# whwh747/A-Low-Texture-Robust-Hybrid-Feature-Based-Visual-Odometry

Measured on AMD Instinct MI355X. Metric: RGB-D frames/sec (640×480, 1k ORB + LSD + PEAC) at 1/2/4/8 GPUs, higher is better.
Workload: dtype u8/u16 integer + f32/f64; 1 GPU; 640x480 synthetic RGB-D, 1000 ORB (quota; 3/4 std + 1/4 lowtex scenes) + LSD lines + PEAC planes, 8192 frames per GPU per step (std640); frames_per_gpu=8192, parallelism=frames sharded, 1 rank(s), no data-path collective, distinct_frames=256, resident_bytes_per_frame_estimate=21100000

## Files before the change

### a-low-texture-robust-hybrid-feature-based-visual-odometry_amd/csrc/orb_level.hip

```cpp
#include "hvo_internal.hpp"
#include <string.h>
#include <algorithm>
#include <vector>

#define LT_TP 64
#define LT_ND (LT_TP / 4)
#define LT_TR 46
#define LT_MAXO 40
#define LT_CAND 368
#define LT_PEND 328
#define LT_TABN 48

typedef unsigned short lt_us2 __attribute__((ext_vector_type(2)));

struct __attribute__((aligned(16))) LtWave {
    uint32_t T[LT_TR * LT_ND];
    union {
        struct { uint8_t S[LT_TR * LT_TP]; unsigned short cand[LT_CAND]; unsigned short pend[LT_PEND]; unsigned long long mk_min[8], mk_ini[8]; } f;
        uint32_t V[((LT_TR + 1) / 2) * LT_MAXO];
    } u;
    int tab[4][LT_TABN];
};
static_assert(sizeof(LtWave) <= 8192, "five workgroups per CU");

struct LevelArgs {
    const uint8_t *rd; size_t rd_stride;
    uint8_t *wr; size_t wr_stride;
    uint8_t *blur; size_t blur_stride;
    LevelGeom L, D; int has_next;
    const OrbTile *tiles; int ntiles, tpw, groups, nframes;
    const int *xofs, *xalpha, *yofs, *ybeta;
    uint32_t *cell_kp; int *cell_cnt; int ncells, iniTh, minTh; int *flags;
    int k0, k1, k2, k3;
    int res_dw;
    int skip;
};

static __device__ __forceinline__ int lt_reflect(int p, int n)
{
    if (p < 0) p = -p;
    if (p >= n) p = 2 * (n - 1) - p;
    return p < 0 ? 0 : p;
}
static __device__ __forceinline__ int lt_mbcnt(unsigned long long m)
{
    return __builtin_amdgcn_mbcnt_hi((unsigned)(m >> 32), __builtin_amdgcn_mbcnt_lo((unsigned)m, 0u));
}

static __device__ __forceinline__ int lt_min3(int a, int b, int c) { int r; asm("v_min3_i32 %0, %1, %2, %3" : "=v"(r) : "v"(a), "v"(b), "v"(c)); return r; }
static __device__ __forceinline__ int lt_max3(int a, int b, int c) { int r; asm("v_max3_i32 %0, %1, %2, %3" : "=v"(r) : "v"(a), "v"(b), "v"(c)); return r; }

static __device__ __forceinline__ int lt_fast_score(const uint8_t *p, int v)
{
    constexpr int tp = LT_TP;
    int r[16];
    r[0] = p[3 * tp];    r[1] = p[3 * tp + 1];   r[2] = p[2 * tp + 2];   r[3] = p[tp + 3];
    r[4] = p[3];         r[5] = p[-tp + 3];      r[6] = p[-2 * tp + 2];  r[7] = p[-3 * tp + 1];
    r[8] = p[-3 * tp];   r[9] = p[-3 * tp - 1];  r[10] = p[-2 * tp - 2]; r[11] = p[-tp - 3];
    r[12] = p[-3];       r[13] = p[tp - 3];      r[14] = p[2 * tp - 2];  r[15] = p[3 * tp - 1];
    int d[16], e[16], a3[16], b3[16];
#pragma unroll
    for (int k = 0; k < 16; k++) { d[k] = v - r[k]; e[k] = r[k] - v; }
#pragma unroll
    for (int k = 0; k < 16; k++) { a3[k] = lt_min3(d[k], d[(k + 1) & 15], d[(k + 2) & 15]); b3[k] = lt_min3(e[k], e[(k + 1) & 15], e[(k + 2) & 15]); }
    int best = -1000;
#pragma unroll
    for (int k = 0; k < 16; k++)
        best = lt_max3(best, lt_min3(a3[k], a3[(k + 3) & 15], a3[(k + 6) & 15]), lt_min3(b3[k], b3[(k + 3) & 15], b3[(k + 6) & 15]));
    return best - 1;
}

static __device__ __forceinline__ void lt_row_sums(unsigned W0, unsigned W1, unsigned W2, unsigned klo, unsigned khi, unsigned hs[4])
{
    const unsigned A0 = __builtin_amdgcn_alignbyte(W1, W0, 1), B0 = __builtin_amdgcn_alignbyte(W2, W1, 1);
    const unsigned A1 = __builtin_amdgcn_alignbyte(W1, W0, 2), B1 = __builtin_amdgcn_alignbyte(W2, W1, 2);
    const unsigned A2 = __builtin_amdgcn_alignbyte(W1, W0, 3), B2 = __builtin_amdgcn_alignbyte(W2, W1, 3);
    hs[0] = __builtin_amdgcn_udot4(A0, klo, __builtin_amdgcn_udot4(B0, khi, 0u, false), false);
    hs[1] = __builtin_amdgcn_udot4(A1, klo, __builtin_amdgcn_udot4(B1, khi, 0u, false), false);
    hs[2] = __builtin_amdgcn_udot4(A2, klo, __builtin_amdgcn_udot4(B2, khi, 0u, false), false);
    hs[3] = __builtin_amdgcn_udot4(W1, klo, __builtin_amdgcn_udot4(W2, khi, 0u, false), false);
}
static __device__ __forceinline__ unsigned lt_dot2(unsigned a, unsigned w, unsigned c)
{
    return __builtin_amdgcn_udot2(__builtin_bit_cast(lt_us2, a), __builtin_bit_cast(lt_us2, w), c, false);
}

template <int NW>
__global__ __launch_bounds__(64 * NW, 5) void k_orb_level(const LevelArgs A)
{
    __shared__ LtWave lds_[NW];
    const int wv = threadIdx.x >> 6, lane = threadIdx.x & 63;
    const int xcd = blockIdx.x & 7, q = blockIdx.x >> 3;
    const int fr8 = q / A.groups, g = q - fr8 * A.groups;
    const int frame = fr8 * 8 + xcd;
    if (frame >= A.nframes) return;
    LtWave &W = lds_[wv];
    const LevelGeom &L = A.L;
    const uint8_t *img = A.rd + (size_t)frame * A.rd_stride;
    uint8_t *bdst = A.blur + (size_t)frame * A.blur_stride;
    const uint8_t *T8 = reinterpret_cast<const uint8_t *>(W.T);
    const unsigned long long ltm = (1ull << lane) - 1ull;

    for (int ti = 0; ti < A.tpw; ti++) {
        const int tidx = (g * A.tpw + ti) * NW + wv;
        if (tidx >= A.ntiles) break;
        const OrbTile t = A.tiles[tidx];
        const int lx0 = t.bx0 - 4, ly0 = t.by0 - 3;
        const int rows = t.bh + 6;
        const int xr = max(t.fx0 + t.fw, t.bx0 + t.bw) + 3;
        __builtin_amdgcn_wave_barrier();
        {
            typedef uint32_t lt_u4 __attribute__((ext_vector_type(4), aligned(4)));
            uint4 v[3];
#pragma unroll
            for (int k = 0; k < 3; k++) {
                const int i = lane + 64 * k, r = i >> 2, c = i & 3;
                v[k] = make_uint4(0, 0, 0, 0);
                if (r < rows) {
                    const int y = lt_reflect(ly0 + r, L.h);
                    const lt_u4 q4 = *reinterpret_cast<const lt_u4 *>(img + (size_t)y * L.pitch + lx0 + 16 * c);
                    v[k] = make_uint4(q4.x, q4.y, q4.z, q4.w);
                }
            }
            int tb0 = 0, tb1 = 0, tb2 = 0, tb3 = 0;
            const bool want_tab = A.has_next && lane < LT_TABN;
            if (want_tab) {
                const int dx = min(t.dxa + lane, A.D.w - 1), dy = min(t.dya + lane, A.D.h - 1);
                tb0 = A.xofs[dx]; tb1 = A.xalpha[dx]; tb2 = A.yofs[dy]; tb3 = A.ybeta[dy];
            }
#pragma unroll
            for (int k = 0; k < 3; k++) {
                const int i = lane + 64 * k;
                if ((i >> 2) < rows) reinterpret_cast<uint4 *>(W.T)[i] = v[k];
            }
            if (want_tab) { W.tab[0][lane] = tb0; W.tab[1][lane] = tb1; W.tab[2][lane] = tb2; W.tab[3][lane] = tb3; }
        }
        if (lx0 < 0) {
            if (lane < rows) { const unsigned d1 = W.T[lane * LT_ND + 1]; W.T[lane * LT_ND] = __builtin_amdgcn_perm(d1, d1, 0x01020300u); }
        }
        if (xr > L.w) {
            uint8_t *Tb = reinterpret_cast<uint8_t *>(W.T);
            if (lane < rows) {
                const int c = L.w - lx0;
#pragma unroll
                for (int k = 0; k < 3; k++) if (L.w + k < xr) Tb[lane * LT_TP + c + k] = Tb[lane * LT_TP + c - 2 - k];
            }
        }
        __builtin_amdgcn_wave_barrier();

        if (t.fw > 0 && !(A.skip & 1)) {
            uint8_t *S = W.u.f.S;
            {
                uint4 *Sz = reinterpret_cast<uint4 *>(S);
                const int nz = (rows * LT_TP + 15) >> 4;
                for (int i = lane; i < nz; i += 64) Sz[i] = make_uint4(0, 0, 0, 0);
            }
            const int cx0 = t.fx0 - lx0, cx1 = cx0 + t.fw, ih = t.bh, iw = t.fw, P = iw * ih;
            const int dws = cx0 >> 2, nd = ((cx1 - 1) >> 2) - dws + 1, items = ih * nd;
            const int rcp = (65536 + nd - 1) / nd;
            const int minTh = A.minTh;
            int ncand = 0, npend = 0;
            auto rest = [&](const unsigned short *pp, int cnt) {
                int pass = 0, xy = 0;
                if (lane < cnt) {
                    xy = pp[lane];
                    const uint8_t *qq = T8 + (xy >> 8) * LT_TP + (xy & 0xFF);
                    const int v = qq[0];
#define LT_PMN(o) min((int)qq[o], (int)qq[-(o)])
#define LT_PMX(o) max((int)qq[o], (int)qq[-(o)])
                    const int n0 = LT_PMN(3 * LT_TP), n1 = LT_PMN(3), n2 = LT_PMN(2 * LT_TP + 2), n3 = LT_PMN(-2 * LT_TP + 2);
                    const int n4 = LT_PMN(3 * LT_TP + 1), n5 = LT_PMN(LT_TP + 3), n6 = LT_PMN(-LT_TP + 3), n7 = LT_PMN(-3 * LT_TP + 1);
                    const int x0 = LT_PMX(3 * LT_TP), x1 = LT_PMX(3), x2 = LT_PMX(2 * LT_TP + 2), x3 = LT_PMX(-2 * LT_TP + 2);
                    const int x4 = LT_PMX(3 * LT_TP + 1), x5 = LT_PMX(LT_TP + 3), x6 = LT_PMX(-LT_TP + 3), x7 = LT_PMX(-3 * LT_TP + 1);
#undef LT_PMN
#undef LT_PMX
                    const int M1 = lt_max3(lt_max3(n0, n1, n2), lt_max3(n3, n4, n5), max(n6, n7));
                    const int M2 = lt_min3(lt_min3(x0, x1, x2), lt_min3(x3, x4, x5), min(x6, x7));
                    pass = (int)(M1 < v - minTh) | (int)(M2 > v + minTh);
                }
                const unsigned long long m = __ballot(pass != 0);
                const int p = ncand + __popcll(m & ltm);
                if (pass && p < LT_CAND) W.u.f.cand[p] = (unsigned short)xy;
                ncand += __popcll(m);
            };
            for (int base = 0; base < items; base += 64) {
                const int it = base + lane;
                const int ok = it < items;
                const int itc = ok ? it : 0;
                const int r = (itc * rcp) >> 16, dwi = dws + itc - r * nd;
                const unsigned t4 = W.T[r * LT_ND + dwi], v4 = W.T[(r + 3) * LT_ND + dwi], b4 = W.T[(r + 6) * LT_ND + dwi];
                const int xb = 4 * dwi;
                const int jl = max(cx0 - xb, 0), jh = min(cx1 - xb, 4);
                const unsigned inm = ok ? (((1u << jh) - 1u) & ~((1u << jl) - 1u)) : 0u;
                int pj[4];
#pragma unroll
                for (int j = 0; j < 4; j++) {
                    const int v = (v4 >> (8 * j)) & 0xFF, tt = (t4 >> (8 * j)) & 0xFF, bb = (b4 >> (8 * j)) & 0xFF;
                    pj[j] = (int)((inm >> j) & 1u) & ((int)(min(tt, bb) < v - minTh) | (int)(max(tt, bb) > v + minTh));
                }
                const unsigned long long m0 = __ballot(pj[0] != 0), m1 = __ballot(pj[1] != 0), m2 = __ballot(pj[2] != 0), m3 = __ballot(pj[3] != 0);
                if ((m0 | m1 | m2 | m3) != 0ull) {
                    const int p0 = npend + lt_mbcnt(m0) + lt_mbcnt(m1) + lt_mbcnt(m2) + lt_mbcnt(m3);
                    const int p1 = p0 + pj[0], p2 = p1 + pj[1], p3 = p2 + pj[2];
                    const int yx = ((r + 3) << 8) | xb;
                    W.u.f.pend[pj[0] ? p0 : LT_PEND - 1] = (unsigned short)yx;
                    W.u.f.pend[pj[1] ? p1 : LT_PEND - 1] = (unsigned short)(yx + 1);
                    W.u.f.pend[pj[2] ? p2 : LT_PEND - 1] = (unsigned short)(yx + 2);
                    W.u.f.pend[pj[3] ? p3 : LT_PEND - 1] = (unsigned short)(yx + 3);
                    npend += __popcll(m0) + __popcll(m1) + __popcll(m2) + __popcll(m3);
                    int head = 0;
                    while (npend - head >= 64) { rest(W.u.f.pend + head, 64); head += 64; }
                    if (head) {
                        const int left = npend - head;
                        const int tv = W.u.f.pend[head + (lane < left ? lane : 0)];
                        if (lane < left) W.u.f.pend[lane] = (unsigned short)tv;
                        npend = left;
                    }
                }
            }
            if (npend > 0) rest(W.u.f.pend, npend);
            __builtin_amdgcn_wave_barrier();
            const uint8_t *T0 = T8 + 3 * LT_TP + cx0;
            uint8_t *S0 = S + 3 * LT_TP + cx0;
            if (ncand <= LT_CAND) {
                for (int i = lane; i < ncand; i += 64) {
                    const int xy = W.u.f.cand[i], o = (xy >> 8) * LT_TP + (xy & 0xFF);
                    const int s = lt_fast_score(T8 + o, T8[o]);
                    S[o] = (uint8_t)(s >= minTh ? s : 0);
                }
            } else {
                for (int p = lane; p < P; p += 64) {
                    const int y = p / iw, x = p - y * iw;
                    const int s = lt_fast_score(T0 + y * LT_TP + x, T0[y * LT_TP + x]);
                    S0[y * LT_TP + x] = (uint8_t)(s >= minTh ? s : 0);
                }
            }
            __builtin_amdgcn_wave_barrier();
            uint32_t *out = A.cell_kp + ((size_t)frame * A.ncells + t.cell) * HVO_CELL_CAP;
            const int ex = lx0 - L.minBX, ey = ly0 - L.minBY;
            int n_ini = 0, pos = 0;
            if (ncand <= LT_CAND) {
                int st = 0;
                for (int base = 0; base < ncand; base += 64, st++) {
                    const int i = base + lane;
// ... 121 lines not shown
                for (int i = 0; i < 4; i++) {
                    sxo[i] = W.tab[0][4 * c + i] - lx0;
                    a01[i] = (unsigned)W.tab[1][4 * c + i];
                }
                const int wbase = sxo[0] >> 2;
                unsigned sel = 0;
#pragma unroll
                for (int i = 0; i < 4; i++) sel |= (unsigned)((sxo[i] - 4 * wbase) & 7) << (8 * i);
                auto hrow = [&](int sy, unsigned tt[4]) {
                    if (A.res_dw) {
                        const uint32_t *rp = W.T + (sy - ly0) * LT_ND + wbase;
                        const uint32_t w0 = rp[0], w1 = rp[1], w2 = rp[2];
                        const uint32_t Lb = __builtin_amdgcn_perm(w1, w0, sel);
                        const uint32_t Rb = __builtin_amdgcn_perm(__builtin_amdgcn_alignbyte(w2, w1, 1), __builtin_amdgcn_alignbyte(w1, w0, 1), sel);
                        tt[0] = lt_dot2(__builtin_amdgcn_perm(Rb, Lb, 0x0c040c00u), a01[0], 0u);
                        tt[1] = lt_dot2(__builtin_amdgcn_perm(Rb, Lb, 0x0c050c01u), a01[1], 0u);
                        tt[2] = lt_dot2(__builtin_amdgcn_perm(Rb, Lb, 0x0c060c02u), a01[2], 0u);
                        tt[3] = lt_dot2(__builtin_amdgcn_perm(Rb, Lb, 0x0c070c03u), a01[3], 0u);
                    } else {
                        const uint8_t *rp = T8 + (sy - ly0) * LT_TP;
#pragma unroll
                        for (int i = 0; i < 4; i++) {
                            const int sx = min(max(sxo[i], 0), LT_TP - 2);
                            tt[i] = lt_dot2((unsigned)rp[sx] | ((unsigned)rp[sx + 1] << 16), a01[i], 0u);
                        }
                    }
                };
#pragma unroll
                for (int rr = 0; rr < RG; rr++) {
                    const int dyu = t.dya + gr * RG + rr, dy = min(dyu, t.dyb - 1);
                    const int yo = W.tab[2][dy - t.dya], sy0 = yo & 0xFFFF, sy1 = yo >> 16;
                    const unsigned yb = (unsigned)W.tab[3][dy - t.dya];
                    const unsigned b0 = yb & 0xFFFFu, b1 = yb >> 16;
                    unsigned t0[4], t1[4];
                    hrow(sy0, t0);
                    hrow(sy1, t1);
                    uint32_t ov = 0;
#pragma unroll
                    for (int i = 0; i < 4; i++) {
                        const unsigned v = ((__umul24(b0, t0[i] >> 4) >> 16) + (__umul24(b1, t1[i] >> 4) >> 16) + 2u) >> 2;
                        ov |= (v & 0xFFu) << (8 * i);
                    }
                    if (dyu < t.dyb) *reinterpret_cast<uint32_t *>(dst + (size_t)dy * D.pitch + dxq) = ov;
                }
            }
        }
    }
}

struct LtIv { int a, b, idx; };

static void lt_split(std::vector<LtIv> &v, int a, int b, int align)
{
    if (b <= a) return;
    const int len = b - a, n = (len + LT_MAXO - 1) / LT_MAXO;
    int step = (len + n - 1) / n;
    step = (step + align - 1) / align * align;
    for (int s = a; s < b; s += step) v.push_back({ s, std::min(s + step, b), -1 });
}

bool orb_level_build(OrbPlan &P, const std::vector<CellDesc> &cells, const std::vector<int> &xofs, const std::vector<int> &yofs, std::vector<OrbTile> &tiles)
{
    tiles.clear();
    for (int l = 0; l < P.nlevels; l++) {
        LevelGeom &L = P.lev[l];
        P.lt_off[l] = (int)tiles.size();
        std::vector<LtIv> cols, rws;
        for (int c = L.cell_off; c < L.cell_off + L.ncells; c++) {
            const CellDesc &cd = cells[c];
            const int fx = cd.x0 + 3, fxe = cd.x0 + cd.vw - 3, fy = cd.y0 + 3, fye = cd.y0 + cd.vh - 3;
            bool hc = false, hr = false;
            for (auto &iv : cols) hc |= iv.a == fx;
            for (auto &iv : rws) hr |= iv.a == fy;
            if (!hc) cols.push_back({ fx, fxe, (int)cols.size() });
            if (!hr) rws.push_back({ fy, fye, (int)rws.size() });
        }
        if ((int)(cols.size() * rws.size()) != L.ncells) return false;
        for (size_t j = 1; j < cols.size(); j++) if (cols[j].a != cols[j - 1].b) return false;
        for (size_t i = 1; i < rws.size(); i++) if (rws[i].a != rws[i - 1].b) return false;
        const int W4 = (L.w + 3) & ~3;
        std::vector<LtIv> xs, ys;
        if (cols.empty()) { lt_split(xs, 0, W4, 4); lt_split(ys, 0, L.h, 1); }
        else {
            lt_split(xs, 0, cols[0].a & ~3, 4);
            for (size_t j = 0; j < cols.size(); j++) {
                const int a = cols[j].a & ~3, b = (j + 1 < cols.size() ? cols[j + 1].a : cols[j].b) & ~3;
                xs.push_back({ a, b, (int)j });
            }
            lt_split(xs, cols.back().b & ~3, W4, 4);
            lt_split(ys, 0, rws[0].a, 1);
            for (size_t i = 0; i < rws.size(); i++) ys.push_back({ rws[i].a, rws[i].b, (int)i });
            lt_split(ys, rws.back().b, L.h, 1);
        }
        const bool has_next = l + 1 < P.nlevels;
        const int *xo = has_next ? xofs.data() + P.lev[l + 1].rs_off : nullptr;
        const int *yo = has_next ? yofs.data() + P.lev[l + 1].ry_off : nullptr;
        const int dw = has_next ? P.lev[l + 1].w : 0, dh = has_next ? P.lev[l + 1].h : 0;
        for (auto &iy : ys) for (auto &ix : xs) {
            OrbTile t; memset(&t, 0, sizeof(t));
            t.bx0 = (short)ix.a; t.bw = (short)(ix.b - ix.a); t.by0 = (short)iy.a; t.bh = (short)(iy.b - iy.a);
            t.cell = -1; t.fx0 = (short)ix.a; t.fw = 0;
            if (ix.idx >= 0 && iy.idx >= 0) {
                t.fx0 = (short)cols[ix.idx].a; t.fw = (short)(cols[ix.idx].b - cols[ix.idx].a);
                t.cell = (short)(L.cell_off + iy.idx * (int)cols.size() + ix.idx);
                const CellDesc &cd = cells[t.cell];
                if (cd.x0 + 3 != t.fx0 || cd.y0 + 3 != t.by0 || cd.vh - 6 != t.bh || cd.vw - 6 != t.fw) return false;
            }
            if (t.bh < 1 || (t.bw < 1 && t.fw < 1)) continue;
            const int xr = std::max(t.fx0 + t.fw, t.bx0 + t.bw) + 3;
            if (t.bw > LT_MAXO || t.bh > LT_MAXO || t.bh + 6 > LT_TR || xr - (t.bx0 - 4) > LT_TP || (t.bw & 3) || (t.bx0 & 3)) return false;
            if (t.fw > 0 && ((t.fw * t.bh + 3) / 4 > LT_CAND + 1000)) return false;
            int dxa = 0, dxb = 0, dya = 0, dyb = 0;
            if (has_next && t.bw > 0) {
                const int dw4 = (dw + 3) & ~3;
                while (dxa < dw4 && xo[std::min(dxa, dw - 1)] < t.bx0) dxa += 4;
                dxb = dxa; while (dxb < dw4 && xo[std::min(dxb, dw - 1)] < t.bx0 + t.bw) dxb += 4;
                while (dya < dh && (yo[dya] & 0xFFFF) < t.by0) dya++;
                dyb = dya; while (dyb < dh && (yo[dyb] & 0xFFFF) < t.by0 + t.bh) dyb++;
                for (int dx = dxa; dx < std::min(dxb, dw); dx++) if (xo[dx] + 1 - (t.bx0 - 4) > LT_TP - 1) return false;
            }
            if (dxb - dxa > LT_TABN || dyb - dya > LT_TABN) return false;
            t.dxa = (short)dxa; t.dxb = (short)dxb; t.dya = (short)dya; t.dyb = (short)dyb;
            tiles.push_back(t);
        }
        P.lt_cnt[l] = (int)tiles.size() - P.lt_off[l];
    }
    return true;
}

int orb_level_run(hvo_ctx *ctx, int c0, int n, hipStream_t st, int k0, int k1, int k2, int k3)
{
    OrbPlan &P = ctx->orb;
    for (int l = 0; l < P.nlevels; l++) {
        LevelArgs A;
        A.L = P.lev[l]; A.has_next = l + 1 < P.nlevels; A.D = P.lev[A.has_next ? l + 1 : l];
        if (l == 0) { A.rd = P.d_pyr + (size_t)c0 * P.pyr_bytes; A.rd_stride = P.pyr_bytes; } else { A.rd = P.d_lvl + A.L.lvl_off; A.rd_stride = P.lvl_bytes; }
        A.wr = P.d_lvl + A.D.lvl_off; A.wr_stride = P.lvl_bytes;
        A.blur = P.d_blur + A.L.img_off; A.blur_stride = P.blur_bytes;
        A.tiles = P.d_ltiles + P.lt_off[l]; A.ntiles = P.lt_cnt[l];
        const int nw = P.lt_nw;
        A.tpw = P.lt_tpw; A.groups = (A.ntiles + nw * A.tpw - 1) / (nw * A.tpw); A.nframes = n;
        A.xofs = P.d_rs_xofs + A.D.rs_off; A.xalpha = P.d_rs_xalpha + A.D.rs_off; A.yofs = P.d_rs_yofs + A.D.ry_off; A.ybeta = P.d_rs_ybeta + A.D.ry_off;
        A.cell_kp = P.d_cell_kp; A.cell_cnt = P.d_cell_cnt; A.ncells = P.ncells; A.iniTh = ctx->p.orb_ini_th_fast; A.minTh = ctx->p.orb_min_th_fast;
        A.res_dw = A.has_next && P.resize_dw[l + 1];
#ifdef HVO_TIMING_KNOBS
        A.skip = getenv("HVO_LT_SKIP") ? atoi(getenv("HVO_LT_SKIP")) : 0;
#else
        A.skip = 0;
#endif
        if (ctx->readings & HVO_READING_BLUR_FLOAT) A.skip |= 2;
        A.flags = P.d_flags + c0; A.k0 = k0; A.k1 = k1; A.k2 = k2; A.k3 = k3;
        if (A.ntiles < 1) continue;
        const int n8 = (n + 7) / 8 * 8;
        if (nw == 1) hipLaunchKernelGGL(k_orb_level<1>, dim3((unsigned)(n8 * A.groups)), dim3(64), 0, st, A);
        else if (nw == 2) hipLaunchKernelGGL(k_orb_level<2>, dim3((unsigned)(n8 * A.groups)), dim3(128), 0, st, A);
        else hipLaunchKernelGGL(k_orb_level<4>, dim3((unsigned)(n8 * A.groups)), dim3(256), 0, st, A);
    }
    return HVO_OK;
}
```

### a-low-texture-robust-hybrid-feature-based-visual-odometry_amd/csrc/peac_slots.inc

```

struct SlDec { int p, K, D, code, moff, mB, r0, r1; };
struct __attribute__((aligned(16))) SlLds { double ps[4][16]; LendRed red[4]; LendWin win[4]; SlDec dec[4]; int ncnt[4]; };
#define SL_SLOT(x) ((x) & 0xFFFF)
#define SL_PACK(label, slot) (((label) << 16) | (slot))

static __device__ __forceinline__ void row_min16x2(double (&k)[2], int (&i)[2])
{
    double g[2] = { k[0], k[1] };
#pragma unroll
    for (int s_ = 0; s_ < 4; s_++) {
        double t[2];
#pragma unroll
        for (int n = 0; n < 2; n++) t[n] = dpp_f64(g[n], g[n], s_);
#pragma unroll
        for (int n = 0; n < 2; n++) g[n] = key_min(t[n], g[n]);
    }
    int c[2];
#pragma unroll
    for (int n = 0; n < 2; n++) c[n] = (k[n] == g[n]) ? i[n] : 0x7FFFFFFF;
#pragma unroll
    for (int s_ = 0; s_ < 4; s_++) {
#pragma unroll
        for (int n = 0; n < 2; n++) { const int t = dpp_i32(c[n], c[n], s_); c[n] = min(c[n], t); }
    }
#pragma unroll
    for (int n = 0; n < 2; n++) { k[n] = g[n]; i[n] = c[n]; }
}

struct TQUpdateS {
    double kk[2], mk[2], kn[2]; int li[2], mi[2], x[2], ln[2], nx;
    __device__ __forceinline__ void issue(const TQueue &Q, const int *lq, int rl, int nx_, int x0, double k0, int l0, int x1, double k1, int l1)
    {
        nx = nx_; x[0] = x0; x[1] = x1; kn[0] = k0; kn[1] = k1; ln[0] = l0; ln[1] = l1;
#pragma unroll
        for (int t = 0; t < 2; t++) {
            kk[t] = TQ_INF; mk[t] = TQ_INF; mi[t] = 0x7FFFFFFF; li[t] = 0x7FFFFFFF;
            if (t < nx) { const int s = (x[t] & ~15) + rl; kk[t] = Q.K[s]; li[t] = lq[s]; const int j = ((x[t] >> 8) << 4) + rl; mk[t] = Q.M1k[j]; mi[t] = Q.M1i[j]; }
        }
    }
    __device__ __forceinline__ int take(const TQueue &Q, int *lq, int rl, bool writer)
    {
#pragma unroll
        for (int t = 0; t < 2; t++) if (writer && t < nx) { Q.K[x[t]] = kn[t]; lq[x[t]] = ln[t]; }
        double bk[2]; int bi[2];
#pragma unroll
        for (int t = 0; t < 2; t++) {
            double k = kk[t]; int i = li[t];
#pragma unroll
            for (int u = 0; u < 2; u++) if (u < nx && ((x[u] ^ x[t]) >> 4) == 0 && (x[u] & 15) == rl) { k = kn[u]; i = ln[u]; }
            if (t >= nx) { k = TQ_INF; i = 0x7FFFFFFF; }
            bk[t] = k; bi[t] = i;
        }
        row_min16x2(bk, bi);
#pragma unroll
        for (int t = 0; t < 2; t++) if (writer && t < nx) { Q.M1k[x[t] >> 4] = bk[t]; Q.M1i[x[t] >> 4] = bi[t]; }
        double sk[2]; int si[2];
#pragma unroll
        for (int t = 0; t < 2; t++) {
            double k = mk[t]; int i = mi[t];
#pragma unroll
            for (int u = 0; u < 2; u++) if (u < nx && ((x[u] ^ x[t]) >> 8) == 0 && ((x[u] >> 4) & 15) == rl) { k = bk[u]; i = bi[u]; }
            if (t >= nx) { k = TQ_INF; i = 0x7FFFFFFF; }
            sk[t] = k; si[t] = i;
        }
        row_min16x2(sk, si);
        double k = TQ_INF; int i = 0x7FFFFFFF;
        for (int j = rl; j < Q.n0; j += 16) {
            double a = Q.M0k[j]; int b = Q.M0i[j];
#pragma unroll
            for (int u = 0; u < 2; u++) if (u < nx && (x[u] >> 8) == j) { a = sk[u]; b = si[u]; }
            if (hless(a, b, k, i)) { k = a; i = b; }
        }
#pragma unroll
        for (int t = 0; t < 2; t++) if (writer && t < nx) { Q.M0k[x[t] >> 8] = sk[t]; Q.M0i[x[t] >> 8] = si[t]; }
        row_min16(k, i);
        return k < TQ_INF ? i : -1;
    }
};

static __device__ __forceinline__ void sl_find8(const int (&u)[8], int n, int x0, int D, int K, int &iD, int &iK)
{
    unsigned mD = 0, mK = 0;
#pragma unroll
    for (int j = 7; j >= 0; j--) { mD = (mD << 1) | (unsigned)(u[j] == D); mK = (mK << 1) | (unsigned)(u[j] == K); }
    const unsigned valid = n >= 8 ? 0xFFu : ((1u << (n < 0 ? 0 : n)) - 1u);
    mD &= valid; mK &= valid;
    if (mD && iD < 0) iD = x0 + __ffs((int)mD) - 1;
    if (mK && iK < 0) iK = x0 + __ffs((int)mK) - 1;
}
static __device__ __forceinline__ void sl_find(const int *pool, int off, int cnt, int D, int K, bool wantK, int &iD, int &iK)
{
    iD = -1; iK = -1;
    for (int x0 = 0; x0 < cnt; x0 += 8) {
        int u[8];
#pragma unroll
        for (int j = 0; j < 8; j++) u[j] = x0 + j < cnt ? pool[off + x0 + j] : -1;
        sl_find8(u, cnt - x0, x0, D, K, iD, iK);
        if (iD >= 0 && (!wantK || iK >= 0)) break;
    }
}

__global__ __launch_bounds__(64) void k_peac_cluster_slots(ClArgs a, int nframes)
{
    constexpr int GL = 16, NG = 4;
    extern __shared__ __attribute__((aligned(16))) unsigned char tq_lds[];
    __shared__ SlLds S;
    const int lane = threadIdx.x, gl = lane & 15, gi = lane >> 4;
    int frame = (a.perm ? a.perm[blockIdx.x] : (int)blockIdx.x) * NG + gi;
    const bool galive = frame < nframes;
    if (!galive) frame = nframes - 1;
    const int nblk = a.nblk, Nw = a.Nw, Nh = a.Nh;
    TQueue Q; Q.n0 = a.tq_n0;
    Q.K = a.tqK + (size_t)frame * Q.n0 * 256; Q.M1k = a.tqM1k + (size_t)frame * Q.n0 * 16; Q.M1i = a.tqM1i + (size_t)frame * Q.n0 * 16;
    Q.M0k = reinterpret_cast<double *>(tq_lds) + (size_t)gi * Q.n0;
    Q.M0i = reinterpret_cast<int *>(tq_lds + (size_t)NG * Q.n0 * sizeof(double)) + (size_t)gi * Q.n0;
    int *lq = a.tqLq + (size_t)frame * Q.n0 * 256;
    Q.n0 = (nblk + 255) >> 8;
    double *segD = a.segD + (size_t)frame * a.segcap * SEG_D;
    int *segI = a.segI + (size_t)frame * a.segcap * SEG_I;
    int *pool = a.pool + (size_t)frame * a.poolcap, *pool2 = a.pool2 + (size_t)frame * a.poolcap;
    int *parent = a.parent + (size_t)frame * nblk, *dsize = a.dsize + (size_t)frame * nblk;
    int *eflag = a.eflag + (size_t)frame * nblk;
    HotNode *hot = a.hot + (size_t)frame * a.segcap;
    PT_DECL
#ifdef HVO_PEAC_TIMING
    const unsigned long long t_in0 = clock64();
#endif
    if (galive) for (int b = gl; b < nblk; b += GL) { parent[b] = b; dsize[b] = 1; if (!a.edges_done) eflag[b] = 0; }
    __syncthreads();
#define GOK(c) (segI[(size_t)(c) * SEG_I + 6] != 0)
#define SD(c) (segD + (size_t)(c) * SEG_D)
    if (galive && !a.edges_done) for (int i = gl; i < Nh; i += GL) {
        for (int j = 1; j < Nw; j += 2) {
            const int c = i * Nw + j;
            if (!GOK(c - 1)) { --j; continue; }
            if (!GOK(c)) continue;
            if (j < Nw - 1 && !GOK(c + 1)) { ++j; continue; }
            const double th = t_ang_init(a, SD(c)[11]);
            if ((j < Nw - 1 && nsim(SD(c - 1), SD(c + 1)) >= th) || (j == Nw - 1 && nsim(SD(c), SD(c - 1)) >= th)) {
                eflag[c] |= 1; eflag[c - 1] |= 2;
                if (j < Nw - 1) { eflag[c] |= 2; eflag[c + 1] |= 1; }
            } else --j;
        }
    }
    __syncthreads();
    if (galive && !a.edges_done) for (int j = gl; j < Nw; j += GL) {
        for (int i = 1; i < Nh; i += 2) {
            const int c = i * Nw + j;
            if (!GOK(c - Nw)) { --i; continue; }
            if (!GOK(c)) continue;
            if (i < Nh - 1 && !GOK(c + Nw)) { ++i; continue; }
            const double th = t_ang_init(a, SD(c)[11]);
            if ((i < Nh - 1 && nsim(SD(c - Nw), SD(c + Nw)) >= th) || (i == Nh - 1 && nsim(SD(c), SD(c - Nw)) >= th)) {
                eflag[c] |= 4; eflag[c - Nw] |= 8;
                if (i < Nh - 1) { eflag[c] |= 8; eflag[c + Nw] |= 4; }
            } else --i;
        }
    }
#undef GOK
#undef SD
    __syncthreads();
    int hn = 0;
    for (int base = 0; base < Q.n0 * 256; base += GL) {
        const int b = base + gl;
        bool ok = false; double mse_b = 0;
        if (galive && b < nblk) {
            const int *si = segI + (size_t)b * SEG_I;
            const int e = eflag[b];
            int n = 0;
            if (e & 4) pool[b * 4 + n++] = b - Nw;
            if (e & 1) pool[b * 4 + n++] = b - 1;
            if (e & 2) pool[b * 4 + n++] = b + 1;
            if (e & 8) pool[b * 4 + n++] = b + Nw;
            ok = si[6] != 0;
            hot[b].cnt = n;
            hot[b].rid = SL_PACK(b, b);
            mse_b = hot[b].mse;
        }
        if (galive) { Q.K[b] = ok ? mse_b : TQ_INF; lq[b] = SL_PACK(b, b); }
        hn += __popcll(Grp<GL>::ballot(ok));
    }
    __syncthreads();
#ifdef HVO_PEAC_TIMING
    const unsigned long long t_in1 = clock64();
#endif
    if (galive) for (int j = gl; j < Q.n0 * 16; j += GL) {
        double k = TQ_INF; int i = 0x7FFFFFFF;
        for (int q = 0; q < 16; q++) { const double kq = Q.K[j * 16 + q]; const int iq = SL_PACK(j * 16 + q, j * 16 + q); if (hless(kq, iq, k, i)) { k = kq; i = iq; } }
        Q.M1k[j] = k; Q.M1i[j] = i;
    }
    __syncthreads();
    for (int j = gl; j < Q.n0; j += GL) {
        double k = TQ_INF; int i = 0x7FFFFFFF;
        if (galive) for (int q = 0; q < 16; q++) { const double kq = Q.M1k[j * 16 + q]; const int iq = Q.M1i[j * 16 + q]; if (hless(kq, iq, k, i)) { k = kq; i = iq; } }
        Q.M0k[j] = k; Q.M0i[j] = i;
    }
#ifdef HVO_PEAC_TIMING
    if (lane == 0) { const unsigned long long t_in2 = clock64(); atomicAdd(&g_peac_t[12], t_in1 - t_in0); atomicAdd(&g_peac_t[13], t_in2 - t_in1); atomicAdd(&g_peac_t[14], 1ull); }
#endif
    int nseg = nblk, pooltop = nblk * 4, next = 0, flags = 0;
    int *ext = a.extracted + (size_t)frame * 2 * MAX_PLANES;
    const unsigned long long lt_mask = (1ull << gl) - 1;
    const unsigned long long wave_lt = (1ull << lane) - 1;
    __syncthreads();
    int ptop = hn > 0 ? tq_top(Q, gl) : -1;
    double nps[9], npn[3]; int n_cnt = 0, n_off = 0, n_N = 0, n_rid = 0, n_dsr = 0, n_dss = 0;
    auto fetch_next = [&](int r) {
        const HotNode *h = hot + (r < 0 ? 0 : SL_SLOT(r));
        n_cnt = h->cnt; n_off = h->off; n_N = h->N; n_rid = h->rid; n_dsr = h->dsr; n_dss = h->dss;
#pragma unroll
        for (int q2 = 0; q2 < 9; q2++) nps[q2] = h->st[q2];
        npn[0] = h->nrm[0]; npn[1] = h->nrm[1]; npn[2] = h->nrm[2];
    };
    int a0n = -1, f_id = -1, fg = gi, nbase = 16; bool lend = false;
    auto assign_and_prefetch = [&]() {
        const int c = hn > 0 ? n_cnt : 0;
        const int c0 = __builtin_amdgcn_readlane(c, 0), c1 = __builtin_amdgcn_readlane(c, 16), c2 = __builtin_amdgcn_readlane(c, 32), c3 = __builtin_amdgcn_readlane(c, 48);
        const int x0 = max(c0 - 16, 0), x1 = max(c1 - 16, 0), x2 = max(c2 - 16, 0), x3 = max(c3 - 16, 0), X = x0 + x1 + x2 + x3;
        a0n = gl < c ? pool[n_off + gl] : -1;
        lend = false; fg = gi; f_id = -1; nbase = 16;
        if (X > 0) {
            const bool idle = gl >= c;
            const unsigned long long im = __ballot(idle);
            const int r = __popcll(im & wave_lt), I = __popcll(im);
            const int b1 = x0, b2 = x0 + x1, b3 = b2 + x2;
            const int g2 = r < b1 ? 0 : r < b2 ? 1 : r < b3 ? 2 : 3;
            const int xb = g2 == 0 ? 0 : g2 == 1 ? b1 : g2 == 2 ? b2 : b3;
            const int myxb = gi == 0 ? 0 : gi == 1 ? b1 : gi == 2 ? b2 : b3, myx = gi == 0 ? x0 : gi == 1 ? x1 : gi == 2 ? x2 : x3;
            nbase = 16 + min(myx, max(I - myxb, 0));
            const unsigned long long fp = __shfl((unsigned long long)(uintptr_t)pool, g2 << 4);
            const int foff = __shfl(n_off, g2 << 4);
            lend = idle && r < X;
            if (lend) { fg = g2; f_id = reinterpret_cast<const int *>((uintptr_t)fp)[foff + 16 + r - xb]; }
        }
    };
    fetch_next(ptop);
    assign_and_prefetch();
    while (__any(hn > 0)) {
        const bool act = hn > 0;
        PT_CNT(8, 1)
        const bool need_gc = act && pooltop > a.poolcap - 2 * a.nblk;
        if (__any(need_gc)) {
            gpool_gc<GL>(hot, nblk, pool, pool2, pooltop, need_gc);
            n_off = hot[ptop < 0 ? 0 : SL_SLOT(ptop)].off;
            assign_and_prefetch();
        }
        PT(0)
        const int p = act ? SL_SLOT(ptop) : -1;
        const bool live = act;
        const int pcnt = live ? n_cnt : 0, poff = n_off, pN = n_N, prid = n_rid & 0xFFFF, pdsr = n_dsr, pdss = n_dss;
        if (gl == 0) {
#pragma unroll
            for (int q = 0; q < 9; q++) S.ps[gi][q] = nps[q];
            S.ps[gi][9] = npn[0]; S.ps[gi][10] = npn[1]; S.ps[gi][11] = npn[2];
            reinterpret_cast<int *>(&S.ps[gi][12])[0] = pN;
            S.ncnt[gi] = -1;
        }
        lend_lds_order();
        const bool anyl = __any(lend);
        const bool home = gl < pcnt;
        const bool c1v = home || lend;
        const int cg = lend ? fg : gi;
        const int nb1 = home ? a0n : f_id;
        const int cframe = __shfl(frame, cg << 4);
        HotNode *hotc = a.hot + (size_t)cframe * a.segcap;
        int *poolc = reinterpret_cast<int *>((uintptr_t)__shfl((unsigned long long)(uintptr_t)pool, cg << 4));
        int id_cur = (nbase + gl < pcnt) ? pool[poff + nbase + gl] : -1;
        double ps_r[9], pn_r[3]; int pNc;
        PT(2)
        int noff1 = 0, ncnt1 = 0, c1N = 0, c1lab = 0; bool c1has = false; double c1m = 0, c1c2 = 0, c1l0 = 0;
        {
            double lst[9]; int lN = 4; bool has = false;
#pragma unroll
            for (int q = 0; q < 9; q++) lst[q] = 0;
            double nst[9], nnr[3]; int nN = 0;
#pragma unroll
            for (int q = 0; q < 9; q++) nst[q] = 0;
            nnr[0] = nnr[1] = nnr[2] = 0;
            if (c1v) {
                const HotNode *nd = hotc + nb1;
                nN = nd->N; noff1 = nd->off; ncnt1 = nd->cnt; c1lab = nd->rid >> 16;
                nnr[0] = nd->nrm[0]; nnr[1] = nd->nrm[1]; nnr[2] = nd->nrm[2];
#pragma unroll
                for (int q = 0; q < 9; q++) nst[q] = nd->st[q];
            }
            {
                const double *pc = S.ps[cg];
#pragma unroll
                for (int q = 0; q < 9; q++) ps_r[q] = pc[q];
                pn_r[0] = pc[9]; pn_r[1] = pc[10]; pn_r[2] = pc[11];
                pNc = reinterpret_cast<const int *>(pc + 12)[0];
            }
            if (c1v && !(fabs(pn_r[0] * nnr[0] + pn_r[1] * nnr[1] + pn_r[2] * nnr[2]) < a.c60)) {
#pragma unroll
                for (int q = 0; q < 9; q++) lst[q] = ps_r[q] + nst[q];
                lN = pNc + nN;
                has = true;
            }
            if (__any(has)) {
                double tc2, tl0, tm;
                PT(2)
                stats_lambda_dev(lst, lN, tc2, tl0, tm);
                PT(4)
                if (has) { c1has = true; c1m = tm; c1c2 = tc2; c1l0 = tl0; c1N = lN; }
            }
        }
        double gmin; int rg, rx, wlab;
        {
            const bool c1own = c1has && !lend;
            gmin = c1own ? c1m : TQ_INF;
#define GM_STEP(o) { const double t = row_partner<o>(gmin); gmin = key_min(t, gmin); }
            GM_STEP(1) GM_STEP(2) GM_STEP(4) GM_STEP(8)
#undef GM_STEP
            double gminc = gmin;
            if (anyl) {
                if (gl == 0) S.red[gi].minbits = (unsigned long long)__double_as_longlong(gmin);
                lend_lds_order();
                if (lend && c1has) atomicMin(&S.red[fg].minbits, (unsigned long long)__double_as_longlong(c1m));
                lend_lds_order();
                gmin = __longlong_as_double((long long)S.red[gi].minbits);
                gminc = __longlong_as_double((long long)S.red[cg].minbits);
            }
            const bool c1good = (double)c1N >= c1m;
            rg = 0x7FFFFFFF; rx = -1;
            if (c1own && c1m == gmin) { if (c1good) rg = c1lab; rx = c1lab; }
#define GM_STEP(o) { const int t0 = row_partner<o>(rg), t1 = row_partner<o>(rx); rg = min(rg, t0); rx = max(rx, t1); }
            GM_STEP(1) GM_STEP(2) GM_STEP(4) GM_STEP(8)
#undef GM_STEP
            if (anyl) {
                if (gl == 0) { S.red[gi].gid = rg; S.red[gi].xid = rx; }
                lend_lds_order();
                if (lend && c1has && c1m == gminc) { if (c1good) atomicMin(&S.red[fg].gid, c1lab); atomicMax(&S.red[fg].xid, c1lab); }
                lend_lds_order();
                rg = S.red[gi].gid; rx = S.red[gi].xid;
            }
            wlab = rg != 0x7FFFFFFF ? rg : rx;
            int wlabc = wlab;
            if (anyl) {
                if (gl == 0) S.red[gi].gid = wlab;
                lend_lds_order();
                wlabc = S.red[cg].gid;
            }
            if (c1has && c1m == gminc && c1lab == wlabc) {
                LendWin &w = S.win[cg];
                w.c2 = c1c2; w.l0 = c1l0; w.noff = noff1; w.ncnt = ncnt1; w.lN = c1N; w.flag = nb1;
            }
        }
        int t_id = -1, t_off = 0, t_cnt = 0;
        if (__any(nbase < pcnt)) {
            if (anyl) {
                const double *pc = S.ps[gi];
#pragma unroll
                for (int q = 0; q < 9; q++) ps_r[q] = pc[q];
                pn_r[0] = pc[9]; pn_r[1] = pc[10]; pn_r[2] = pc[11];
            }
            for (int base = nbase; __any(base < pcnt); base += GL) {
                PT_CNT(9, 1)
                const int k = base + gl;
                const int id_nxt = k + GL < pcnt ? pool[poff + k + GL] : -1;
                double lst[9]; int lN = 4, nb = 0, noff_ = 0, ncnt_ = 0, lab = 0; bool has = false;
#pragma unroll
                for (int q = 0; q < 9; q++) lst[q] = 0;
                if (k < pcnt) {
                    nb = id_cur;
                    const HotNode *nd = hot + nb;
                    const int nN = nd->N; noff_ = nd->off; ncnt_ = nd->cnt; lab = nd->rid >> 16;
                    if (base == nbase) { t_id = nb; t_off = noff_; t_cnt = ncnt_; }
                    if (!(fabs(pn_r[0] * nd->nrm[0] + pn_r[1] * nd->nrm[1] + pn_r[2] * nd->nrm[2]) < a.c60)) {
#pragma unroll
                        for (int q = 0; q < 9; q++) lst[q] = ps_r[q] + nd->st[q];
                        lN = pN + nN;
                        has = true;
                    }
                }
                if (__any(has)) {
                    double tc2, tl0, tm;
                    PT(2)
// ... 7 lines not shown
                    int prg = tied && good ? lab : 0x7FFFFFFF, prx = tied ? lab : -1;
#define GM_STEP(o) { const int t0 = row_partner<o>(prg), t1 = row_partner<o>(prx); prg = min(prg, t0); prx = max(prx, t1); }
                    GM_STEP(1) GM_STEP(2) GM_STEP(4) GM_STEP(8)
#undef GM_STEP
                    if (pm < gmin) { gmin = pm; rg = prg; rx = prx; }
                    else if (pm == gmin) { rg = min(rg, prg); rx = max(rx, prx); }
                    const int nw = rg != 0x7FFFFFFF ? rg : rx;
                    if (nw != wlab && tied && tm == gmin && lab == nw) {
                        LendWin &w = S.win[gi];
                        w.c2 = tc2; w.l0 = tl0; w.noff = noff_; w.ncnt = ncnt_; w.lN = lN; w.flag = nb;
                    }
                    wlab = nw;
                }
                id_cur = id_nxt;
            }
        }
        PT(2)
        lend_lds_order();
        const bool any_cand = gmin < TQ_INF;
        const double m = gmin, c2 = S.win[gi].c2, l0 = S.win[gi].l0; int noff = S.win[gi].noff, ncnt = S.win[gi].ncnt; const int wN = S.win[gi].lN, nb = S.win[gi].flag;
        PT(3)
        bool do_merge = false;
        if (live && any_cand) {
            const double t = 1.6e-6 * c2 * c2 + 8.0;
            if (m < t * t) {
                if (nseg >= a.segcap || pooltop + pcnt + ncnt > a.poolcap) flags |= 8;
                else do_merge = true;
            }
        }
        if (!do_merge) ncnt = 0;
        const int id = nseg;
        const bool no_merge = live && !do_merge;
        if (do_merge) { PT_CNT(10, 1) nseg++; }
        if (no_merge) { PT_CNT(11, 1) }
        PT(4)
        const bool kp = pcnt >= ncnt;
        const int K = do_merge ? (kp ? p : nb) : -1, D = do_merge ? (kp ? nb : p) : p;
        const int moff = pooltop;
        if (act) hn -= 1;
        int p_c = p, K_c = K, D_c = D, moff_c = moff; bool dm_c = do_merge, nm_c = no_merge, kp_c = kp;
        if (anyl) {
            if (gl == 0) { SlDec &d = S.dec[gi]; d.p = p; d.K = K; d.D = D; d.code = (do_merge ? 1 : 0) | (no_merge ? 2 : 0) | (kp ? 4 : 0); d.moff = moff; }
            lend_lds_order();
            if (lend) { const SlDec &d = S.dec[fg]; p_c = d.p; K_c = d.K; D_c = d.D; moff_c = d.moff; dm_c = (d.code & 1) != 0; nm_c = (d.code & 2) != 0; kp_c = (d.code & 4) != 0; }
        }
        TQUpdateS qu;
        const int aid = c1v ? nb1 : -1, aoff = noff1, acnt = ncnt1;
        const bool editA = aid >= 0 && (nm_c || (dm_c && !kp_c && aid != K_c));
        const bool anyA = __any(editA);
        ListFind fa; fa.off = 0; fa.cnt = 0;
#pragma unroll
        for (int j = 0; j < 8; j++) fa.u[j] = -1;
        if (anyA) fa.issue(poolc, aoff, editA ? acnt : 0);
        const int vB = gl < ncnt ? pool[noff + gl] : -1;
        qu.issue(Q, lq, gl, act ? (do_merge ? 2 : 1) : 0, D, TQ_INF, 0x7FFFFFFF, K < 0 ? 0 : K, m, SL_PACK(id, K < 0 ? 0 : K));
        const bool inB = vB >= 0 && vB != p;
        const bool editB = inB && kp;
        int qb_off = 0, qb_cnt = 0;
        if (editB) { qb_off = hot[vB].off; qb_cnt = hot[vB].cnt; }
        ptop = qu.take(Q, lq, gl, gl == 0);
        if (hn <= 0) ptop = -1;
        const int ptslot = ptop < 0 ? -1 : SL_SLOT(ptop);
        const int ptslot_c = anyl ? __shfl(ptslot, cg << 4) : ptslot;
        PT(1)
        fetch_next(ptop);
        const bool anyB = __any(editB);
        ListFind fb; fb.off = 0; fb.cnt = 0;
#pragma unroll
        for (int j = 0; j < 8; j++) fb.u[j] = -1;
        if (anyB) fb.issue(pool, qb_off, editB ? qb_cnt : 0);
        int a_iD = -1, a_iK = -1;
        if (anyA) {
            const int wantK = dm_c;
            sl_find8(fa.u, fa.cnt, 0, p_c, wantK ? K_c : p_c, a_iD, a_iK);
            bool more = fa.cnt > 8 && !(a_iD >= 0 && (!wantK || a_iK >= 0));
            for (int x0 = 8; __any(more); x0 += 8) {
                int w[8];
#pragma unroll
                for (int j = 0; j < 8; j++) w[j] = (more && x0 + j < fa.cnt) ? poolc[fa.off + x0 + j] : -1;
                if (more) sl_find8(w, fa.cnt - x0, x0, p_c, wantK ? K_c : p_c, a_iD, a_iK);
                more = more && x0 + 8 < fa.cnt && !(a_iD >= 0 && (!wantK || a_iK >= 0));
            }
        }
        int mcnt = 0;
        {
            int b_iD = -1, b_iK = -1;
            if (editB) {
                sl_find8(fb.u, fb.cnt, 0, nb, p, b_iD, b_iK);
                if (fb.cnt > 8 && !(b_iD >= 0 && b_iK >= 0)) {
                    for (int x0 = 8; x0 < fb.cnt; x0 += 8) {
                        int w[8];
#pragma unroll
                        for (int j = 0; j < 8; j++) w[j] = x0 + j < fb.cnt ? pool[fb.off + x0 + j] : -1;
                        sl_find8(w, fb.cnt - x0, x0, nb, p, b_iD, b_iK);
                        if (b_iD >= 0 && b_iK >= 0) break;
                    }
                }
            }
            bool keep = inB && !kp;
            if (editB) {
                if (b_iK >= 0) {
                    if (b_iD >= 0) { if (b_iD != qb_cnt - 1) pool[qb_off + b_iD] = pool[qb_off + qb_cnt - 1]; hot[vB].cnt = qb_cnt - 1; if (vB == ptslot) S.ncnt[gi] = qb_cnt - 1; }
                } else { if (b_iD >= 0) pool[qb_off + b_iD] = p; keep = true; }
            }
            const unsigned long long km = Grp<GL>::ballot(keep);
            if (keep) pool[moff + mcnt + __popcll(km & lt_mask)] = vB;
            mcnt += __popcll(km);
        }
        PT(5)
        for (int base = GL; __any(base < ncnt); base += GL) {
            const int k = base + gl;
            int v = -1; bool keep = false;
            if (k < ncnt) {
                v = pool[noff + k];
                if (v != p) {
                    if (!kp) keep = true;
                    else {
                        const int off = hot[v].off, cnt = hot[v].cnt;
                        int iD, iK;
                        sl_find(pool, off, cnt, nb, p, true, iD, iK);
                        if (iK >= 0) { if (iD >= 0) { if (iD != cnt - 1) pool[off + iD] = pool[off + cnt - 1]; hot[v].cnt = cnt - 1; if (v == ptslot) S.ncnt[gi] = cnt - 1; } }
                        else { if (iD >= 0) pool[off + iD] = p; keep = true; }
                    }
                }
            }
            const unsigned long long km = Grp<GL>::ballot(keep);
            if (keep) pool[moff + mcnt + __popcll(km & lt_mask)] = v;
            mcnt += __popcll(km);
        }
        PT(6)
        if (__any(aid >= 0)) {
            bool keep = aid >= 0 && dm_c && kp_c && aid != D_c;
            if (editA) {
                HotNode *hv = hotc + aid;
                const int off = aoff, cnt = acnt;
                if (dm_c && a_iK < 0) { if (a_iD >= 0) poolc[off + a_iD] = K_c; keep = true; }
                else if (a_iD >= 0) {
                    if (a_iD != cnt - 1) poolc[off + a_iD] = poolc[off + cnt - 1];
                    hv->cnt = cnt - 1;
                    if (aid == ptslot_c) S.ncnt[cg] = cnt - 1;
                }
            }
            if (!anyl) {
                const unsigned long long km = Grp<GL>::ballot(keep);
                if (keep) pool[moff + mcnt + __popcll(km & lt_mask)] = aid;
                mcnt += __popcll(km);
            } else {
                if (gl == 0) S.dec[gi].mB = mcnt;
                lend_lds_order();
                const int mB_c = lend ? S.dec[fg].mB : mcnt;
                const unsigned long long km = __ballot(keep);
                const unsigned long long s0 = __ballot(c1v && cg == 0), s1 = __ballot(c1v && cg == 1), s2 = __ballot(c1v && cg == 2), s3 = __ballot(c1v && cg == 3);
                const unsigned long long sc_ = cg == 0 ? s0 : cg == 1 ? s1 : cg == 2 ? s2 : s3, so_ = gi == 0 ? s0 : gi == 1 ? s1 : gi == 2 ? s2 : s3;
                if (keep) poolc[moff_c + mB_c + __popcll(km & sc_ & wave_lt)] = aid;
                mcnt += __popcll(km & so_);
            }
        }
        PT(5)
        for (int base = nbase; __any(live && base < pcnt); base += GL) {
            const int k = base + gl;
            int v = -1; bool keep = false;
            if (live && k < pcnt) {
                const bool first = base == nbase;
                v = first ? t_id : pool[poff + k];
                if (do_merge && kp) keep = v != nb;
                else if (!do_merge || v != nb) {
                    HotNode *hv = hot + v;
                    int off = t_off, cnt = t_cnt;
                    if (!first) { off = hv->off; cnt = hv->cnt; }
                    int iD, iK;
                    sl_find(pool, off, cnt, p, do_merge ? nb : p, do_merge, iD, iK);
                    if (do_merge && iK < 0) { if (iD >= 0) pool[off + iD] = nb; keep = true; }
                    else if (iD >= 0) { if (iD != cnt - 1) pool[off + iD] = pool[off + cnt - 1]; hv->cnt = cnt - 1; if (v == ptslot) S.ncnt[gi] = cnt - 1; }
                }
            }
            const unsigned long long km = Grp<GL>::ballot(keep);
            if (keep) pool[moff + mcnt + __popcll(km & lt_mask)] = v;
            mcnt += __popcll(km);
        }
        PT(6)
        if (__any(do_merge)) {
            const HotNode *W = hot + (do_merge ? nb : 0);
            const double *pc = S.ps[gi];
            double mst[9], mn[3];
#pragma unroll
            for (int q = 0; q < 9; q++) mst[q] = pc[q] + W->st[q];
            const int WN = W->N, Wrid = W->rid & 0xFFFF, bdss = W->dss, bdsr = W->dsr;
            const int bN = do_merge ? wN : 4;
            stats_vector_dev(mst, bN, l0, mn);
            if (do_merge && gl == 0) {
                HotNode *M = hot + K;
#pragma unroll
                for (int q = 0; q < 9; q++) M->st[q] = mst[q];
                M->nrm[0] = mn[0]; M->nrm[1] = mn[1]; M->nrm[2] = mn[2]; M->mse = m;
                int root = pdsr, size = pdss + bdss;
                if (pdsr == bdsr) size = pdss;
                else if (pdss < bdss) { parent[pdsr] = bdsr; dsize[bdsr] = size; root = bdsr; }
                else { parent[bdsr] = pdsr; dsize[pdsr] = size; }
                M->N = bN; M->rid = SL_PACK(id, pN >= WN ? prid : Wrid); M->off = moff; M->cnt = mcnt; M->dss = size; M->dsr = root;
                hot[D].cnt = 0;
            }
        }
        if (do_merge) pooltop += pcnt + ncnt;
        if (no_merge) {
            if (pN >= MIN_SUPPORT) { if (next < MAX_PLANES) { if (gl == 0) ext[next] = p; next++; } else flags |= 16; }
            if (gl == 0) hot[p].cnt = 0;
        }
        PT(7)
        __syncthreads();
        {
            const bool fresh = do_merge && ptslot == K;
            if (__any(fresh)) { if (fresh) fetch_next(ptop); }
            lend_lds_order();
            { const int e = S.ncnt[gi]; if (e >= 0) n_cnt = e; }
            if (fresh) { n_cnt = mcnt; n_off = moff; }
            assign_and_prefetch();
        }
        PT(0)
    }
    __syncthreads();
    if (gl == 0) {
        for (int i = 1; i < next; i++) {
            int v = ext[i], j = i - 1;
            int vN = hot[v].N;
            while (j >= 0 && hot[ext[j]].N < vN) { ext[j + 1] = ext[j]; j--; }
            ext[j + 1] = v;
        }
    }
    __syncthreads();
    for (int v = a.nblk + gl; v < nseg; v += GL) { int *si = segI + (size_t)v * SEG_I; si[2] = 1; si[3] = 0; si[4] = 0; }
    __syncthreads();
    {
        int lab[(MAX_PLANES + GL - 1) / GL];
        for (int e = gl, q = 0; e < next; e += GL, q++) {
            const int s = ext[e]; const HotNode *nv = hot + s;
            const int v = nv->rid >> 16;
            lab[q] = v;
            double *sd = segD + (size_t)v * SEG_D; int *si = segI + (size_t)v * SEG_I;
            const double sc = 1.0 / nv->N;
#pragma unroll
            for (int q2 = 0; q2 < 9; q2++) sd[q2] = nv->st[q2];
            sd[9] = nv->st[0] * sc; sd[10] = nv->st[1] * sc; sd[11] = nv->st[2] * sc;
            sd[12] = nv->nrm[0]; sd[13] = nv->nrm[1]; sd[14] = nv->nrm[2]; sd[15] = nv->mse;
            si[0] = nv->N; si[1] = nv->rid & 0xFFFF; si[2] = 0; si[3] = 0; si[4] = 0; si[5] = 0; si[6] = 1; si[7] = 0;
        }
        __syncthreads();
        for (int e = gl, q = 0; e < next; e += GL, q++) ext[e] = lab[q];
    }
    __syncthreads();
    PT(0)
    PT_FLUSH
    if (galive && gl == 0) {
        int *meta = a.meta + (size_t)frame * 16;
        meta[0] = nseg; meta[1] = 0; meta[2] = next; meta[3] = flags; meta[6] = 0;
    }
}
```

Baseline: 60160 frames/s.

## Simplify FAST score via ring min/max, retune occupancy, use dynamic LDS and mbcnt

The FAST corner score is recomputed as arc-wise max/min of ring pixels relative to the center. This drops the per-pixel difference arrays and about halves the min3/max3 work. The ORB level kernel moves to dynamic shared memory, forces 6 waves per EU, and makes the wave index scalar via readfirstlane. The PEAC cluster kernel gets a 3-waves-per-EU hint and replaces popcount-of-masked-ballot with mbcnt. Forcing occupancy may cause register spills, and the equivalence of the new score formula must hold exactly.

After: 60920 frames/s, median of 6. +1.3%, better.

```diff
diff --git a/a-low-texture-robust-hybrid-feature-based-visual-odometry_amd/csrc/orb_level.hip b/a-low-texture-robust-hybrid-feature-based-visual-odometry_amd/csrc/orb_level.hip
--- a/a-low-texture-robust-hybrid-feature-based-visual-odometry_amd/csrc/orb_level.hip
+++ b/a-low-texture-robust-hybrid-feature-based-visual-odometry_amd/csrc/orb_level.hip
@@ -58,16 +58,26 @@
     r[4] = p[3];         r[5] = p[-tp + 3];      r[6] = p[-2 * tp + 2];  r[7] = p[-3 * tp + 1];
     r[8] = p[-3 * tp];   r[9] = p[-3 * tp - 1];  r[10] = p[-2 * tp - 2]; r[11] = p[-tp - 3];
     r[12] = p[-3];       r[13] = p[tp - 3];      r[14] = p[2 * tp - 2];  r[15] = p[3 * tp - 1];
-    int d[16], e[16], a3[16], b3[16];
-#pragma unroll
-    for (int k = 0; k < 16; k++) { d[k] = v - r[k]; e[k] = r[k] - v; }
-#pragma unroll
-    for (int k = 0; k < 16; k++) { a3[k] = lt_min3(d[k], d[(k + 1) & 15], d[(k + 2) & 15]); b3[k] = lt_min3(e[k], e[(k + 1) & 15], e[(k + 2) & 15]); }
-    int best = -1000;
-#pragma unroll
-    for (int k = 0; k < 16; k++)
-        best = lt_max3(best, lt_min3(a3[k], a3[(k + 3) & 15], a3[(k + 6) & 15]), lt_min3(b3[k], b3[(k + 3) & 15], b3[(k + 6) & 15]));
-    return best - 1;
+    int lo, hi;
+    {
+        int x3[16];
+#pragma unroll
+        for (int k = 0; k < 16; k++) x3[k] = lt_max3(r[k], r[(k + 1) & 15], r[(k + 2) & 15]);
+        lo = lt_max3(x3[0], x3[3], x3[6]);
+#pragma unroll
+        for (int k = 1; k < 15; k += 2) lo = lt_min3(lo, lt_max3(x3[k], x3[(k + 3) & 15], x3[(k + 6) & 15]), lt_max3(x3[k + 1], x3[(k + 4) & 15], x3[(k + 7) & 15]));
+        lo = min(lo, lt_max3(x3[15], x3[2], x3[5]));
+    }
+    {
+        int n3[16];
+#pragma unroll
+        for (int k = 0; k < 16; k++) n3[k] = lt_min3(r[k], r[(k + 1) & 15], r[(k + 2) & 15]);
+        hi = lt_min3(n3[0], n3[3], n3[6]);
+#pragma unroll
+        for (int k = 1; k < 15; k += 2) hi = lt_max3(hi, lt_min3(n3[k], n3[(k + 3) & 15], n3[(k + 6) & 15]), lt_min3(n3[k + 1], n3[(k + 4) & 15], n3[(k + 7) & 15]));
+        hi = max(hi, lt_min3(n3[15], n3[2], n3[5]));
+    }
+    return max(v - lo, hi - v) - 1;
 }
 
 static __device__ __forceinline__ void lt_row_sums(unsigned W0, unsigned W1, unsigned W2, unsigned klo, unsigned khi, unsigned hs[4])
@@ -86,10 +96,12 @@
 }
 
 template <int NW>
-__global__ __launch_bounds__(64 * NW, 5) void k_orb_level(const LevelArgs A)
-{
-    __shared__ LtWave lds_[NW];
-    const int wv = threadIdx.x >> 6, lane = threadIdx.x & 63;
+__attribute__((amdgpu_waves_per_eu(6, 6)))
+__global__ __launch_bounds__(64 * NW) void k_orb_level(const LevelArgs A)
+{
+    extern __shared__ __attribute__((aligned(16))) unsigned char lt_lds_[];
+    LtWave *lds_ = reinterpret_cast<LtWave *>(lt_lds_);
+    const int wv = __builtin_amdgcn_readfirstlane((int)(threadIdx.x >> 6)), lane = threadIdx.x & 63;
     const int xcd = blockIdx.x & 7, q = blockIdx.x >> 3;
     const int fr8 = q / A.groups, g = q - fr8 * A.groups;
     const int frame = fr8 * 8 + xcd;
@@ -517,9 +529,9 @@
         A.flags = P.d_flags + c0; A.k0 = k0; A.k1 = k1; A.k2 = k2; A.k3 = k3;
         if (A.ntiles < 1) continue;
         const int n8 = (n + 7) / 8 * 8;
-        if (nw == 1) hipLaunchKernelGGL(k_orb_level<1>, dim3((unsigned)(n8 * A.groups)), dim3(64), 0, st, A);
-        else if (nw == 2) hipLaunchKernelGGL(k_orb_level<2>, dim3((unsigned)(n8 * A.groups)), dim3(128), 0, st, A);
-        else hipLaunchKernelGGL(k_orb_level<4>, dim3((unsigned)(n8 * A.groups)), dim3(256), 0, st, A);
+        if (nw == 1) hipLaunchKernelGGL(k_orb_level<1>, dim3((unsigned)(n8 * A.groups)), dim3(64), 1 * sizeof(LtWave), st, A);
+        else if (nw == 2) hipLaunchKernelGGL(k_orb_level<2>, dim3((unsigned)(n8 * A.groups)), dim3(128), 2 * sizeof(LtWave), st, A);
+        else hipLaunchKernelGGL(k_orb_level<4>, dim3((unsigned)(n8 * A.groups)), dim3(256), 4 * sizeof(LtWave), st, A);
     }
     return HVO_OK;
 }
diff --git a/a-low-texture-robust-hybrid-feature-based-visual-odometry_amd/csrc/peac_slots.inc b/a-low-texture-robust-hybrid-feature-based-visual-odometry_amd/csrc/peac_slots.inc
--- a/a-low-texture-robust-hybrid-feature-based-visual-odometry_amd/csrc/peac_slots.inc
+++ b/a-low-texture-robust-hybrid-feature-based-visual-odometry_amd/csrc/peac_slots.inc
@@ -77,6 +77,11 @@
         return k < TQ_INF ? i : -1;
     }
 };
+
+static __device__ __forceinline__ int sl_below(unsigned long long m)
+{
+    return (int)__builtin_amdgcn_mbcnt_hi((unsigned)(m >> 32), __builtin_amdgcn_mbcnt_lo((unsigned)m, 0u));
+}
 
 static __device__ __forceinline__ void sl_find8(const int (&u)[8], int n, int x0, int D, int K, int &iD, int &iK)
 {
@@ -100,6 +105,7 @@
     }
 }
 
+__attribute__((amdgpu_waves_per_eu(3, 3)))
 __global__ __launch_bounds__(64) void k_peac_cluster_slots(ClArgs a, int nframes)
 {
     constexpr int GL = 16, NG = 4;
@@ -201,7 +207,6 @@
     int nseg = nblk, pooltop = nblk * 4, next = 0, flags = 0;
     int *ext = a.extracted + (size_t)frame * 2 * MAX_PLANES;
     const unsigned long long lt_mask = (1ull << gl) - 1;
-    const unsigned long long wave_lt = (1ull << lane) - 1;
     __syncthreads();
     int ptop = hn > 0 ? tq_top(Q, gl) : -1;
     double nps[9], npn[3]; int n_cnt = 0, n_off = 0, n_N = 0, n_rid = 0, n_dsr = 0, n_dss = 0;
@@ -222,7 +227,7 @@
         if (X > 0) {
             const bool idle = gl >= c;
             const unsigned long long im = __ballot(idle);
-            const int r = __popcll(im & wave_lt), I = __popcll(im);
+            const int r = sl_below(im), I = __popcll(im);
             const int b1 = x0, b2 = x0 + x1, b3 = b2 + x2;
             const int g2 = r < b1 ? 0 : r < b2 ? 1 : r < b3 ? 2 : 3;
             const int xb = g2 == 0 ? 0 : g2 == 1 ? b1 : g2 == 2 ? b2 : b3;
@@ -536,7 +541,7 @@
                 const unsigned long long km = __ballot(keep);
                 const unsigned long long s0 = __ballot(c1v && cg == 0), s1 = __ballot(c1v && cg == 1), s2 = __ballot(c1v && cg == 2), s3 = __ballot(c1v && cg == 3);
                 const unsigned long long sc_ = cg == 0 ? s0 : cg == 1 ? s1 : cg == 2 ? s2 : s3, so_ = gi == 0 ? s0 : gi == 1 ? s1 : gi == 2 ? s2 : s3;
-                if (keep) poolc[moff_c + mB_c + __popcll(km & sc_ & wave_lt)] = aid;
+                if (keep) poolc[moff_c + mB_c + sl_below(km & sc_)] = aid;
                 mcnt += __popcll(km & so_);
             }
         }
```
